# LumiOwO/RT-Octree

Hardware: AMD Instinct MI355X
Metric: FPS @ 800x800 (Lego SPP=6) + PSNR vs ref; 1/2/4/8 GPU scaling (higher is better)
Workload: dtype f32 (traversal, filter) + f16 x f16 -> f32 (GuidanceNet conv, fused MFMA kernel); 1 GPU; configs[1]: lego-like synthetic PlenOctree SH16 (2122333 nodes, depth 10), 800x800 SPP=6 + GuidanceNet(8,32,5,2,4) denoise, 1 step = 12 launch groups of 100 frames, frames sharded frame g -> rank g mod N; tree_nodes=2122333, frames_per_group=100, streams=2, scenes=1, scene_map=pose, filter=factorised, maps=fp16 packed, parallelism=frames x1, lean_outputs=True, lean_level=2, world=1, gpus_visible=1, launcher=none, full=False

## Files before the change

### rt-octree_amd/csrc/host/tree_layout.cpp

```cpp
#include "host/tree_layout.h"

#include <cmath>
#include <cstring>

#include "host/n3tree_host.h"
#include "rto_tree_bits.h"

namespace rto {

float half_to_float(uint16_t h) {
    const uint32_t sign = (uint32_t)(h & 0x8000u) << 16, exp = (h >> 10) & 0x1fu, man = h & 0x3ffu;
    uint32_t bits;
    if (exp == 0) {
        if (man == 0) {
            bits = sign;
        } else {
            int e = -1;
            uint32_t m = man;
            do {
                ++e;
                m <<= 1;
            } while (!(m & 0x400u));
            bits = sign | (uint32_t)(127 - 15 - e) << 23 | (m & 0x3ffu) << 13;
        }
    } else if (exp == 31) {
        bits = sign | 0x7f800000u | man << 13;
    } else {
        bits = sign | (exp + 127 - 15) << 23 | man << 13;
    }
    float f;
    std::memcpy(&f, &bits, 4);
    return f;
}

bool culling_cells(const int32_t* child, int64_t capacity, const float scale[3], const float offset[3], const uint16_t* sigma,
                   size_t stride, std::vector<float>& out) {
    auto density = [&](int64_t sl) { return half_to_float(sigma[(size_t)sl * stride]); };
    std::vector<uint8_t> lvl((size_t)capacity, 255), has((size_t)capacity, 0);
    std::vector<uint32_t> cx((size_t)capacity, 0), cy((size_t)capacity, 0), cz((size_t)capacity, 0);
    lvl[0] = 0;
    for (int64_t n = 0; n < capacity; ++n) {
        if (lvl[(size_t)n] == 255) continue;
        for (int s = 0; s < 8; ++s) {
            const int32_t c = child[n * 8 + s];
            if (c == 0) continue;
            const int64_t t = n + c;
            if (t <= n || t >= capacity || lvl[(size_t)n] >= 30) return false;
            lvl[(size_t)t] = (uint8_t)(lvl[(size_t)n] + 1);
            cx[(size_t)t] = cx[(size_t)n] * 2 + ((s >> 2) & 1);
            cy[(size_t)t] = cy[(size_t)n] * 2 + ((s >> 1) & 1);
            cz[(size_t)t] = cz[(size_t)n] * 2 + (s & 1);
        }
    }
    for (int64_t n = capacity - 1; n >= 0; --n) {
        if (lvl[(size_t)n] == 255) continue;
        uint8_t h = 0;
        for (int s = 0; s < 8 && !h; ++s) {
            const int32_t c = child[n * 8 + s];
            h = c ? has[(size_t)(n + c)] : (uint8_t)(density(n * 8 + s) > 0.f);
        }
        has[(size_t)n] = h;
    }
    out.clear();
    const float margin = 1e-4f;
    for (int64_t n = 0; n < capacity; ++n) {
        if (lvl[(size_t)n] == 255 || !has[(size_t)n]) continue;
        const int ls = lvl[(size_t)n] + 1;
        if (ls > kOccLevel) continue;
        for (int s = 0; s < 8; ++s) {
            const int32_t c = child[n * 8 + s];
            const bool emit = c ? (ls == kOccLevel && has[(size_t)(n + c)]) : density(n * 8 + s) > 0.f;
            if (!emit) continue;
            const double size = std::ldexp(1.0, -ls);
            const uint32_t q[3] = {cx[(size_t)n] * 2 + ((s >> 2) & 1), cy[(size_t)n] * 2 + ((s >> 1) & 1), cz[(size_t)n] * 2 + (s & 1)};
            for (int i = 0; i < 3; ++i) {
                const double ct = (q[i] + 0.5) * size;
                out.push_back((float)((ct - offset[i]) / scale[i]));
            }
            out.push_back((float)(0.5 * size + margin));
        }
    }
    return true;
}

std::vector<int64_t> bfs_order(const int32_t* child, int64_t capacity, int64_t N3) {
    std::vector<int64_t> order;
    order.reserve((size_t)capacity);
    std::vector<uint8_t> seen((size_t)capacity, 0);
    order.push_back(0);
    seen[0] = 1;
    for (size_t h = 0; h < order.size(); ++h) {
        const int64_t o = order[h];
        for (int64_t s = 0; s < N3; ++s) {
            const int32_t c = child[o * N3 + s];
            if (c == 0) continue;
            const int64_t t = o + c;
            if (!seen[(size_t)t]) {
                seen[(size_t)t] = 1;
                order.push_back(t);
            }
        }
    }
    for (int64_t o = 0; o < capacity; ++o)
        if (!seen[(size_t)o]) order.push_back(o);
    return order;
}

void relay_tree(const std::vector<int64_t>& order, const int32_t* child, const uint16_t* data, int64_t capacity, int64_t N3,
                int data_dim, const HostTree* quant, Relaid& out) {
    std::vector<int64_t> new_of_old((size_t)capacity);
    for (int64_t n = 0; n < capacity; ++n) new_of_old[(size_t)order[(size_t)n]] = n;
    out.child.resize((size_t)(capacity * N3));
// ... 156 lines not shown
```

### rt-octree_amd/csrc/host/tree_layout.h

```cpp
#pragma once
#include <cstddef>
#include <cstdint>
#include <vector>

namespace rto {
struct HostTree;
}

#pragma GCC visibility push(hidden)
namespace rto {

float half_to_float(uint16_t h);

bool culling_cells(const int32_t* child, int64_t capacity, const float scale[3], const float offset[3], const uint16_t* sigma,
                   size_t stride, std::vector<float>& out);

std::vector<int64_t> bfs_order(const int32_t* child, int64_t capacity, int64_t N3);

struct Relaid {
    std::vector<int32_t> child;
    std::vector<uint16_t> data, q_map, q_sigma, q_retained;
};
void relay_tree(const std::vector<int64_t>& order, const int32_t* child, const uint16_t* data, int64_t capacity, int64_t N3,
                int data_dim, const HostTree* quant, Relaid& out);

struct WideImage {
    std::vector<uint32_t> widew, worig, gslot;
    uint32_t n_wide = 0, grid_nodes = 0;
};
bool build_wide_image(const int32_t* child, int64_t capacity, int G, const uint16_t* sigma, size_t stride,
                      WideImage& out);

void wide_image_lookup(const WideImage& wi, const int32_t* child, int G, const uint32_t* points, int64_t n, int32_t* out_level,
                       int64_t* out_slot, uint16_t* out_sigma);

}
#pragma GCC visibility pop
```

### rt-octree_amd/csrc/render_kernels.hip

```cpp
#include <hip/hip_runtime.h>

#include "rto_kernel_types.h"
#include "rto_tree_device.h"

#pragma clang fp contract(off)

#include "rto_render_shared.h"
#include "rto_render_internal.h"

namespace rto {



constexpr int kMarkCells = 2048, kMarkLdsWords = 8192;
template <class MarkFn>
RTO_DEV void mark_cell(const float4 cell, const TreeDev& tree, const FrameDesc& fd, const FrameBatch& fb, MarkFn mark);
template <bool LDS_MASK>
__global__ void __launch_bounds__(256) mark_tiles_kernel(const TreeDev tree, const FrameBatch fb, uint32_t* __restrict__ mask) {
    extern __shared__ uint32_t s_mask[];
    const FrameDesc& fd = fb.f[blockIdx.y];
    uint32_t* const gm = mask + (size_t)blockIdx.y * fb.mask_words;
    if (LDS_MASK) {
        for (int i = threadIdx.x; i < fb.mask_words; i += 256) s_mask[i] = 0u;
        __syncthreads();
    }
    static_assert(kMarkCells % 256 == 0, "a run per thread");
    for (int i = 0; i < kMarkCells / 256; ++i) {
        const int c = (int)blockIdx.x * kMarkCells + (int)threadIdx.x * (kMarkCells / 256) + i;
        if (c >= tree.n_occ_cells) break;
        if (LDS_MASK)
            mark_cell(tree.occ_cells[c], tree, fd, fb, [&](uint32_t w, uint32_t bits) { atomicOr(&s_mask[w], bits); });
        else
            mark_cell(tree.occ_cells[c], tree, fd, fb, [&](uint32_t w, uint32_t bits) { atomicOr(gm + w, bits); });
    }
    if (LDS_MASK) {
        __syncthreads();
        for (int i = threadIdx.x; i < fb.mask_words; i += 256)
            if (s_mask[i]) atomicOr(gm + i, s_mask[i]);
    }
}

template <class MarkFn>
RTO_DEV void mark_cell(const float4 cell, const TreeDev& tree, const FrameDesc& fd, const FrameBatch& fb, MarkFn mark) {
    {
    const float* m = fd.transform;
    const float p[3] = {cell.x - m[9], cell.y - m[10], cell.z - m[11]};
    const float c12[3] = {m[4] * m[8] - m[5] * m[7], m[5] * m[6] - m[3] * m[8], m[3] * m[7] - m[4] * m[6]};
    const float c20[3] = {m[7] * m[2] - m[8] * m[1], m[8] * m[0] - m[6] * m[2], m[6] * m[1] - m[7] * m[0]};
    const float c01[3] = {m[1] * m[5] - m[2] * m[4], m[2] * m[3] - m[0] * m[5], m[0] * m[4] - m[1] * m[3]};
    const float det = m[0] * c12[0] + m[1] * c12[1] + m[2] * c12[2];
    const float inv = 1.f / det;
    const float a = (p[0] * c12[0] + p[1] * c12[1] + p[2] * c12[2]) * inv;
    const float b = (p[0] * c20[0] + p[1] * c20[1] + p[2] * c20[2]) * inv;
    const float d = -(p[0] * c01[0] + p[1] * c01[1] + p[2] * c01[2]) * inv;
    const float frob = sqrtf(c12[0] * c12[0] + c12[1] * c12[1] + c12[2] * c12[2] + c20[0] * c20[0] + c20[1] * c20[1] + c20[2] * c20[2] +
                             c01[0] * c01[0] + c01[1] * c01[1] + c01[2] * c01[2]) * fabsf(inv);
    const float hw[3] = {cell.w / fabsf(tree.scale[0]), cell.w / fabsf(tree.scale[1]), cell.w / fabsf(tree.scale[2])};
    const float r = sqrtf(hw[0] * hw[0] + hw[1] * hw[1] + hw[2] * hw[2]) * 1.001f * frob * 1.0001f;
    if (d <= -r) return;
    const float fx = fabsf(fd.fx), fy = fabsf(fd.fy);
    const bool sphere = d > 2.f * r;
    float x0f = 0.f, x1f = 0.f, y0f = 0.f, y1f = 0.f;
    if (sphere) {
        const float xs = a / d, ys = b / d;
        const float k = r / (d - r);
        const float pxc = 0.5f * fb.width + fd.fx * xs, pyc = 0.5f * fb.height - fd.fy * ys;
        const float rx = fx * k * (1.f + fabsf(xs)) + 1.5f, ry = fy * k * (1.f + fabsf(ys)) + 1.5f;
        x0f = floorf((pxc - rx) * 0.125f), x1f = floorf((pxc + rx) * 0.125f);
        y0f = floorf((pyc - ry) * 0.125f), y1f = floorf((pyc + ry) * 0.125f);
    }
    const float ua[3] = {hw[0] * c12[0] * inv, hw[1] * c12[1] * inv, hw[2] * c12[2] * inv};
    const float ub[3] = {hw[0] * c20[0] * inv, hw[1] * c20[1] * inv, hw[2] * c20[2] * inv};
    const float ud[3] = {-hw[0] * c01[0] * inv, -hw[1] * c01[1] * inv, -hw[2] * c01[2] * inv};
    const float e = 1e-5f * ((fabsf(p[0]) + fabsf(p[1]) + fabsf(p[2])) * frob + r);
    const float dmin = 100.f * e;
    bool front = true, behind = true;
    float xlo = 3e38f, xhi = -3e38f, ylo = 3e38f, yhi = -3e38f;
#pragma unroll
    for (int s = 0; s < 8; ++s) {
        const float sx = (s & 4) ? 1.f : -1.f, sy = (s & 2) ? 1.f : -1.f, sz = (s & 1) ? 1.f : -1.f;
        const float A = a + sx * ua[0] + sy * ua[1] + sz * ua[2];
        const float B = b + sx * ub[0] + sy * ub[1] + sz * ub[2];
        const float D = d + sx * ud[0] + sy * ud[1] + sz * ud[2];
        const float x = A / D, y = B / D, k = e / (D - e);
        const float kx = k * (1.f + fabsf(x)), ky = k * (1.f + fabsf(y));
        front = front && D > dmin && fabsf(x) + fabsf(y) < 3e38f;
        behind = behind && D < -e;
        xlo = fminf(xlo, x - kx), xhi = fmaxf(xhi, x + kx);
        ylo = fminf(ylo, y - ky), yhi = fmaxf(yhi, y + ky);
    }
    if (behind) return;
    const float px0 = 0.5f * fb.width + fd.fx * xlo, px1 = 0.5f * fb.width + fd.fx * xhi;
    const float py0 = 0.5f * fb.height - fd.fy * ylo, py1 = 0.5f * fb.height - fd.fy * yhi;
    const bool box = front && fabsf(px0) + fabsf(px1) + fabsf(py0) + fabsf(py1) < 3e38f;
    if (!box && !sphere) {
        mark((uint32_t)fb.mask_words - 1u, 1u);
        return;
    }
    if (box) {
        const float bx0 = floorf((fminf(px0, px1) - 1.5f) * 0.125f), bx1 = floorf((fmaxf(px0, px1) + 1.5f) * 0.125f);
        const float by0 = floorf((fminf(py0, py1) - 1.5f) * 0.125f), by1 = floorf((fmaxf(py0, py1) + 1.5f) * 0.125f);
        x0f = sphere ? fmaxf(x0f, bx0) : bx0, x1f = sphere ? fminf(x1f, bx1) : bx1;
        y0f = sphere ? fmaxf(y0f, by0) : by0, y1f = sphere ? fminf(y1f, by1) : by1;
    }
    const int tiles_x = (fb.width + 7) >> 3, tiles_y = (fb.height + 7) >> 3;
    if (!(x1f >= 0.f && y1f >= 0.f && x0f < (float)tiles_x && y0f < (float)tiles_y)) {
        if (!(x0f == x0f && y0f == y0f)) mark((uint32_t)fb.mask_words - 1u, 1u);
        return;
    }
    const int x0 = x0f < 0.f ? 0 : (int)x0f, x1 = x1f >= (float)tiles_x ? tiles_x - 1 : (int)x1f;
    const int y0 = y0f < 0.f ? 0 : (int)y0f, y1 = y1f >= (float)tiles_y ? tiles_y - 1 : (int)y1f;
    for (int ty = y0; ty <= y1; ++ty)
        for (int tx = x0; tx <= x1; ++tx) {
            const uint32_t t = (uint32_t)(ty * tiles_x + tx);
            mark(t >> 5, 1u << (t & 31u));
        }
    }
}

__global__ void __launch_bounds__(256) mark_tiles_one_kernel(const TreeDev tree, const FrameDesc fd, const int width, const int height,
                                                             const int mask_words, uint32_t* __restrict__ mask) {
    extern __shared__ uint32_t s_mask[];
    FrameBatch fb;
    fb.width = width;
    fb.height = height;
    fb.mask_words = mask_words;
    const bool lds = mask_words <= kMarkLdsWords;
    if (lds) {
        for (int i = threadIdx.x; i < mask_words; i += 256) s_mask[i] = 0u;
        __syncthreads();
    }
    for (int i = 0; i < kMarkCells / 256; ++i) {
        const int c = (int)blockIdx.x * kMarkCells + (int)threadIdx.x * (kMarkCells / 256) + i;
        if (c >= tree.n_occ_cells) break;
        if (lds)
            mark_cell(tree.occ_cells[c], tree, fd, fb, [&](uint32_t w, uint32_t bits) { atomicOr(&s_mask[w], bits); });
        else
            mark_cell(tree.occ_cells[c], tree, fd, fb, [&](uint32_t w, uint32_t bits) { atomicOr(mask + w, bits); });
    }
    if (lds) {
        __syncthreads();
        for (int i = threadIdx.x; i < mask_words; i += 256)
            if (s_mask[i]) atomicOr(mask + i, s_mask[i]);
    }
}

RTO_DEV bool tile_marked(const FrameBatch& fb, int frame, uint32_t tile_index) {
    const uint32_t* fm = fb.tile_mask + (size_t)frame * fb.mask_words;
    return ((fm[tile_index >> 5] >> (tile_index & 31u)) | fm[fb.mask_words - 1]) & 1u;
}

RTO_DEV bool queue_slot(const FrameBatch& fb, int k, uint32_t pt, uint32_t& entry) {
    const uint32_t qt0 = (uint32_t)fb.qstart[k], qtiles = (uint32_t)fb.qstart[k + 1] - qt0, n = (uint32_t)fb.n;
    if (pt >= qtiles * n) return false;
    uint32_t tile, frame;
    if (fb.tile_major) {
        const uint32_t t = pt / n;
        frame = pt - t * n;
        tile = qt0 + t;
    } else {
        frame = pt / qtiles;
        tile = qt0 + (pt - frame * qtiles);
    }
    const uint32_t tiles_x = (uint32_t)(fb.width + 7) >> 3;
    uint32_t tx, ty;
    if (fb.tile_order) {
        const uint32_t code = fb.tile_order[tile];
        ty = code >> 16;
        tx = code & 0xffffu;
    } else {
        ty = tile / tiles_x;
// ... 290 lines not shown
```

### rt-octree_amd/csrc/rto_abi.cpp

```cpp
#include <algorithm>
#include <cmath>
#include <cstdio>
#include <cstring>
#include <fstream>
#include <sstream>

#include "host/mini_json.h"
#include "rto_denoise_launch.h"
#include "rto_internal.h"

namespace {
thread_local std::string g_err;
}

int set_err(int code, const std::string& msg) {
    g_err = msg;
    return code;
}

namespace {

void pcg_seed(rto::Pcg32& r, uint64_t initstate, uint64_t initseq) {
    auto next = [&]() { r.state = r.state * rto::kPcgMult + r.inc; };
    r.state = 0U;
// ... 411 lines not shown
    if (!c || n < 1 || first_slot < 0 || first_slot + n > c->frames) return 0;
    int lean = 0;
    for (int i = first_slot; i < first_slot + n; ++i) lean += c->lean_slot[(size_t)i] ? 1 : 0;
    return lean == n ? 1 : lean == 0 ? 0 : -1;
}

int rto_ctx_set_tuning(rto_ctx* c, const char* key, int value) {
    if (!c || !key) return set_err(RTO_E_INVALID, "rto_ctx_set_tuning: null argument");
    const std::string k(key);
    if (k == "tile_order") {
        c->tile_order_on = value != 0;
    } else if (k == "xcd_queues") {
        c->xcd_queues = value != 0;
    } else if (k == "tile_major") {
        c->tile_major = value != 0;
    } else if (k == "tile_block") {
        if (value < 1 || value > 64) return set_err(RTO_E_INVALID, "tile_block must be 1..64");
        c->tile_block = value;
        DeviceGuard guard(c->device);
        if (hipDeviceSynchronize() != hipSuccess) return set_err(RTO_E_HIP, "hipDeviceSynchronize failed");
        return build_tile_tables(c);
    } else if (k == "queue_bands") {
        if (value < 0 || value > 64) return set_err(RTO_E_INVALID, "queue_bands must be 0..64");
        c->queue_bands = value;
        DeviceGuard guard(c->device);
        if (hipDeviceSynchronize() != hipSuccess) return set_err(RTO_E_HIP, "hipDeviceSynchronize failed");
        return build_tile_tables(c);
    } else if (k == "refill") {
        c->refill = value;
    } else if (k == "wide_bits") {
        c->test_wide_bits = value;
    } else if (k == "cull") {
        c->cull_on = value != 0;
    } else if (k == "cull_single") {
        c->cull_single = value != 0;
    } else if (k == "frame_via_batch") {
        c->frame_via_batch = value != 0;
    } else if (k == "blocks_per_cu") {
        if (value < 0 || value > 8) return set_err(RTO_E_INVALID, "blocks_per_cu must be 0..8");
        c->occ.cap = value;
    } else if (k == "batch_fallback") {
        c->batch_fallback = value;
    } else if (k == "ray_order") {
        if (value < 0 || value > 1) return set_err(RTO_E_INVALID, "ray_order must be 0 or 1");
        c->ray_order = value;
    } else if (k == "strip_rows") {
        if (value < 1) return set_err(RTO_E_INVALID, "strip_rows must be >= 1");
        c->strip_rows = value;
    } else {
        return set_err(RTO_E_INVALID, "unknown tuning key '" + k + "'");
    }
    return RTO_OK;
}

int rto_ctx_kernel_timing(rto_ctx* c, int enable) {
    if (!c) return set_err(RTO_E_INVALID, "rto_ctx_kernel_timing: null context");
    DeviceGuard guard(c->device);
    if (enable && c->kt_ev.empty()) {
        c->kt_ev.resize((size_t)kKtRing * 4);
        for (auto& e : c->kt_ev) HIP_TRY(hipEventCreate(&e));
    }
    c->kt_on = enable != 0;
    c->kt_count = 0;
    return RTO_OK;
}

// ... 255 lines not shown
```

### rt-octree_amd/csrc/rto_internal.h

```cpp
#pragma once
#include <hip/hip_runtime.h>

#include <algorithm>
#include <atomic>
#include <cmath>
#include <cstring>
#include <mutex>
#include <string>
#include <vector>

#include "rto.h"
#include "rto_abi_common.h"
#include "rto_launch.h"

#pragma GCC visibility push(hidden)

constexpr const char* kNoDeviceMsg = "no HIP device available (librto has no CPU fallback)";
constexpr int kKtRing = 256;
constexpr int kProbeFloats = 128;
#pragma GCC visibility pop

struct rto_tree {
    int device = 0;
    rto::TreeDev dev{};
    rto_tree_info info{};
    void* d_data = nullptr;
    void* d_child = nullptr;
    void* d_nodew = nullptr;
    void* d_topgrid = nullptr;
    void *d_widew = nullptr, *d_worig = nullptr, *d_grid2 = nullptr;
    void* d_shrec = nullptr;
    void* d_recidx = nullptr;
    void* d_occ = nullptr;
    void* d_qrec = nullptr;
    void* d_qcolors = nullptr;
    void* d_qsigma = nullptr;
    void* d_extra = nullptr;
    bool quant = false;
    int flags = 0;
    bool fast_ok = false;
    std::atomic<bool> reference_dropped{false};
    int shrec_halves = 0;
    std::mutex rebuild_mutex;
};

#ifndef RTO_QUEUE_BANDS_DEFAULT
#define RTO_QUEUE_BANDS_DEFAULT 3
#endif
#ifndef RTO_RAY_ORDER_DEFAULT
#define RTO_RAY_ORDER_DEFAULT 0
#endif
struct rto_ctx {
    int device = 0;
    int width = 0, height = 0;
    int frames = 1;
    int sel = 0;
    int num_cus = 256;
    unsigned long long* queue = nullptr;
    rto::FrameDesc* d_frames = nullptr;
    rto::OccupancyCache occ;
    uint32_t* tile_order = nullptr;
    uint32_t* wedge_order = nullptr;
    int wedge_start[rto::kMaxQueues + 1] = {0};
    bool xcd_queues = true;
    bool tile_major = true;
    int tile_block = 4;
    int queue_bands = RTO_QUEUE_BANDS_DEFAULT;
    uint32_t* hits = nullptr;
    int hits_spp = 0;
    uint32_t* tile_mask = nullptr;
    uint32_t* qlist = nullptr;
    uint32_t* qscratch = nullptr;
    int mask_words = 0, q_chunks_cap = 0;
    bool cull_on = true;
    bool frame_via_batch = false;
    int last_n_queues = 0;
    int64_t last_slots = 0;
    int batch_fallback = 0;
    int lean = 0;
    std::vector<uint8_t> lean_slot;
    int test_wide_bits = 0;
    bool cull_single = false;
    int marks_n = 0, marks_slot0 = 0;
    float marks_bg = 0.f;
    bool kt_on = false;
    std::vector<hipEvent_t> kt_ev;
    int kt_count = 0;
    float* aux = nullptr;
    float* noisy = nullptr;
    float* image = nullptr;
    const float* layer_depth = nullptr;
    const float* layer_color = nullptr;
    float* depth = nullptr;
    float* t_near = nullptr;
    int depth_mode = 0;
    float* probe_coeffs = nullptr;
    uint8_t* rgba8 = nullptr;
    rto::Pcg32 rng{};
    rto::PcgJumpEntry* jump = nullptr;
    uint64_t jump_inc = 0;
    bool jump_valid = false;
    int kernel = RTO_KERNEL_AUTO;
    int strip_rows = 1;
    int ray_order = RTO_RAY_ORDER_DEFAULT;
    int refill = 0;
    bool tile_order_on = true;
    bool stats_on = false;
// ... 92 lines not shown
```

### rt-octree_amd/csrc/rto_render_abi.cpp

```cpp
#include <algorithm>
#include <cstring>

#include "rto_internal.h"

namespace {

int ensure_jump_table(rto_ctx* c) {
    if (c->jump_valid && c->jump_inc == c->rng.inc) return RTO_OK;
    std::vector<rto::PcgJumpEntry> tab(4 * 256);
    for (int ch = 0; ch < 4; ++ch)
        for (int j = 0; j < 256; ++j) tab[ch * 256 + j] = pcg_jump(c->rng.inc, (uint64_t)j << (8 * ch));
    if (!c->jump) HIP_TRY(hipMalloc((void**)&c->jump, tab.size() * sizeof(rto::PcgJumpEntry)));
    HIP_TRY(hipMemcpy(c->jump, tab.data(), tab.size() * sizeof(rto::PcgJumpEntry), hipMemcpyHostToDevice));
    c->jump_inc = c->rng.inc;
    c->jump_valid = true;
    return RTO_OK;
}


int check_tree_options(const rto_tree* tree, const rto_options* o, const rto_ctx* ctx) {
    if (!spp_supported(o->spp))
        return set_err(RTO_E_SPP, "spp == " + std::to_string(o->spp) + " not supported. (supported: 1,2,3,4,6,8,16,32)");
    if (tree->device != ctx->device) return set_err(RTO_E_INVALID, "tree and context live on different devices");
    if (tree->d_recidx && !(o->sigma_thresh >= 0.f))
// ... 254 lines not shown
    const bool depth_batched = ctx->depth && ctx->depth_mode == RTO_DEPTH_BATCHED;
    const bool batched = spp_supported(o->spp) && fast_path_for_spp(tree, o->spp, ctx->test_wide_bits, &tdev) != 0 &&
                         ctx->batch_fallback != 1 && (!ctx->depth || depth_batched);
    int rc = check_batch(tree, cams, n, o, ctx, slot0, batched);
    if (rc != RTO_OK) return rc;
    DeviceGuard guard(ctx->device);
    if (!guard.ok) return set_err(RTO_E_HIP, "hipSetDevice failed");
    hipStream_t stream = (hipStream_t)stream_;
    if (ctx->depth && !batched) return depth_frames(tree, cams, rng_jumps, n, o, ctx, stream, slot0);
    if (!batched) return generic_frames(tree, cams, rng_jumps, n, o, ctx, stream, slot0);

    ctx->marks_n = 0;
    for (int f = 0; f < n; ++f) ctx->lean_slot[(size_t)(slot0 + f)] = 0;
    const size_t px = frame_px(ctx);
    if (ctx->hits_spp < o->spp) {
        if (ctx->hits) {
            HIP_TRY(hipDeviceSynchronize());
            HIP_TRY(hipFree(ctx->hits));
            ctx->hits = nullptr;
        }
        HIP_TRY(hipMalloc((void**)&ctx->hits, (size_t)ctx->frames * o->spp * px * sizeof(uint32_t)));
        ctx->hits_spp = o->spp;
    }
    rto::FrameBatch fb;
    std::memset(&fb, 0, sizeof(fb));
    fb.n = n;
    fb.width = ctx->width;
    fb.height = ctx->height;
    rc = queue_layout(ctx, n, &fb);
    if (rc != RTO_OK) return rc;
    ctx->last_n_queues = fb.n_queues;
    ctx->last_slots = (int64_t)tiles_of(ctx) * n;
    const bool cull = ctx->cull_on && tree->dev.occ_cells && o->sigma_thresh >= 0.f && !(tree->dev.ndc_width > 0.f);
    rto::FrameDesc frames[rto::kMaxBatch];
    fb.f = ctx->d_frames;
    fb.lean = o->denoise ? ctx->lean : 0;
    for (int f = 0; f < n; ++f) {
        rto::FrameDesc& d = frames[f];
        d.fx = cams[f].fx;
        d.fy = cams[f].fy;
        std::memcpy(d.transform, cams[f].transform, sizeof(d.transform));
        const rto::Pcg32 rng = rng_after(ctx, frame_jump(rng_jumps, f));
        d.rng_state = rng.state;
        d.rng_inc = rng.inc;
        const rto::FrameOut fo = frame_out(ctx, slot0 + f, o->denoise);
        d.aux = fo.aux;
        d.image = fo.image;
        d.hits = ctx->hits + (size_t)(slot0 + f) * o->spp * px;
    }
    rc = ensure_jump_table(ctx);
    if (rc != RTO_OK) return rc;
    const rto::OptDev od = make_opt_dev(o);
    HIP_TRY(rto::launch_write_frames(frames, n, ctx->d_frames, stream));
    hipEvent_t* ev = nullptr;
    if (ctx->kt_on && ctx->kt_count < kKtRing) ev = &ctx->kt_ev[(size_t)ctx->kt_count++ * 4];
    ctx->occ.force_lds_refusal = ctx->batch_fallback == 2;
    rto::LayerDev layers;
    const bool layered = ctx_layers_at(ctx, slot0, &layers);
    rto::DepthOut dout;
    const bool with_depth = ctx_depth_at(ctx, slot0, &dout);
    hipError_t e = rto::launch_render_batch(o->spp, tdev, od, fb, ctx->jump, ctx->queue,
                                            frames[0].hits,
                                            ctx->num_cus, ctx->refill, cull, &ctx->occ, ev, layered ? &layers : nullptr,
                                            with_depth ? &dout : nullptr, stream);
    if (ctx->occ.lds_refused) {
        if (ev) --ctx->kt_count;
// ... 27 lines not shown
    rto::LayerDev layers;
    const bool layered = ctx_layers_at(ctx, ctx->sel, &layers);
    int rc = check_layers(tree, ctx, layered);
    if (rc == RTO_OK) rc = check_depth(tree, o, ctx);
    if (rc != RTO_OK) return rc;
    if (tree->quant) {
        if (ctx->kernel == RTO_KERNEL_GENERIC || ctx->stats_on)
            return set_err(RTO_E_UNSUPPORTED, "a quantised tree loaded with RTO_TREE_QUANT_DIRECT has no generic kernel / work counters");
        return launch_batch_at(tree, cam, nullptr, 1, o, ctx, stream_, ctx->sel);
    }
    rc = check_tree_options(tree, o, ctx);
    if (rc == RTO_OK) rc = check_camera(*cam, ctx);
    if (rc == RTO_OK && o->enable_probe) rc = probe_check(tree, o, ctx, layered);
    int kernel;
    rto::TreeDev tdev;
    if (rc == RTO_OK) rc = choose_kernel(tree, o, ctx, &kernel, &tdev);
    if (rc != RTO_OK) return rc;
    const bool fast = kernel == RTO_KERNEL_FAST;
    if (fast && ctx->frame_via_batch && ctx->kernel == RTO_KERNEL_AUTO && !ctx->stats_on && !ctx->depth)
        return launch_batch_at(tree, cam, nullptr, 1, o, ctx, stream_, ctx->sel);

    DeviceGuard guard(ctx->device);
    if (!guard.ok) return set_err(RTO_E_HIP, "hipSetDevice failed");
    hipStream_t stream = (hipStream_t)stream_;
    rc = fast ? ensure_jump_table(ctx) : ensure_reference_arrays(tree);
    if (rc != RTO_OK) return rc;
    const rto::CamDev cd = cam_dev(*cam);
    rto::FrameOut fo = frame_out(ctx, ctx->sel, o->denoise);
    const bool cull_one = fast && !ctx->stats_on && ctx->cull_on && ctx->cull_single && tree->dev.occ_cells &&
                          o->sigma_thresh >= 0.f && !(tree->dev.ndc_width > 0.f) && !o->enable_probe;
    if (cull_one) {
        rc = ensure_tile_buffers(ctx, mask_words_of(ctx), 0);
        if (rc != RTO_OK) return rc;
        HIP_TRY(rto::launch_mark_tiles_one(tdev, cd, ctx->tile_mask, ctx->mask_words, stream));
        fo.cull_marks = ctx->tile_mask;
        fo.cull_mask_words = ctx->mask_words;
    }
    bool keep_marks = false;
    if (ctx->stats_on) {
        if (!fast) return set_err(RTO_E_UNSUPPORTED, "work counters need the fast kernel");
        fo.stats = ctx->stats;
        if (ctx->stats_marks) {
            if (ctx->marks_n < 1 || !ctx->tile_mask || ctx->sel < ctx->marks_slot0 || ctx->sel >= ctx->marks_slot0 + ctx->marks_n)
                return set_err(RTO_E_INVALID, "rto_ctx_enable_stats(2): the selected frame slot holds no tile marks of a batched launch");
            fo.stat_marks = ctx->tile_mask + (size_t)(ctx->sel - ctx->marks_slot0) * ctx->mask_words;
            fo.stat_mask_words = ctx->mask_words;
            keep_marks = true;
        }
    }
    if (!keep_marks) ctx->marks_n = 0;
    ctx->lean_slot[(size_t)ctx->sel] = 0;
    rto::DepthOut depth;
    const bool with_depth = ctx_depth_at(ctx, ctx->sel, &depth);
    rc = render_frame(tree, fast ? tdev : tree->dev, kernel, cd, o, make_opt_dev(o), ctx->rng, fo, layered ? &layers : nullptr,
                      with_depth ? &depth : nullptr, ctx, stream);
    if (rc != RTO_OK) return rc;
    if (cull_one && !(layered && layers.color)) {
        ctx->marks_n = 1;
        ctx->marks_slot0 = ctx->sel;
        ctx->marks_bg = o->background_brightness;
    }
    return RTO_OK;
}

int rto_launch_renderer_batch(const rto_tree* tree, const rto_camera* cams, const int64_t* rng_jumps, int n,
                              const rto_options* o, rto_ctx* ctx, void* stream_) {
// ... 60 lines not shown
```

### rt-octree_amd/csrc/rto_tree.cpp

```cpp
#include <algorithm>
#include <cmath>
#include <cstdio>
#include <cstdlib>
#include <cstring>

#include "host/n3tree_host.h"
#include "host/tree_layout.h"
#include "rto_internal.h"

namespace {

bool tree_alloc(rto_tree* t, void** p, size_t bytes) {
    if (hipMalloc(p, bytes) != hipSuccess) return false;
    t->info.device_bytes += (int64_t)bytes;
    return true;
}
void tree_release(rto_tree* t, void** p, size_t bytes) {
    if (!*p) return;
    (void)hipFree(*p);
    *p = nullptr;
    t->info.device_bytes -= (int64_t)bytes;
}

struct HostArrays {
// ... 93 lines not shown
                    tree_alloc(t, &t->d_qrec, rec_b) &&
                    rto::launch_pack_quant((const uint16_t*)tmp_map, (const uint16_t*)tmp_ret, n_slots, nr, nq, q_rec,
                                           (uint16_t*)t->d_qrec, nullptr) == hipSuccess &&
                    hipDeviceSynchronize() == hipSuccess;
    if (tmp_map) (void)hipFree(tmp_map);
    if (tmp_ret) (void)hipFree(tmp_ret);
    if (!ok) return set_err(RTO_E_HIP, "quantised tree upload failed");
    t->quant = true;
    t->dev.q_retain = nr;
    t->dev.q_rec = q_rec;
    return RTO_OK;
}

int build_nodew(rto_tree* t, const HostArrays& h) {
    if (!(h.N == 2 && h.max_depth <= 24 && h.n_slots < (int64_t(1) << rto::kGridSlotBits))) return RTO_OK;
    int* d_bad = nullptr;
    if (!tree_alloc(t, &t->d_nodew, (size_t)h.n_slots * 4) || hipMalloc((void**)&d_bad, 4) != hipSuccess ||
        hipMemset(d_bad, 0, 4) != hipSuccess)
        return set_err(RTO_E_HIP, "hipMalloc(nodew) failed");
    const uint16_t* d_sigma = h.quant ? (const uint16_t*)t->d_qsigma : (const uint16_t*)t->d_data;
    hipError_t e = rto::launch_build_nodew((const int32_t*)t->d_child, d_sigma, h.n_slots, h.quant ? 1 : h.data_dim,
                                           (uint32_t*)t->d_nodew, d_bad, nullptr);
    int bad = 0;
    if (e == hipSuccess) e = hipMemcpy(&bad, d_bad, 4, hipMemcpyDeviceToHost);
    (void)hipFree(d_bad);
    if (e != hipSuccess) return hip_fail("build_nodew failed: ", e);
    t->fast_ok = !bad;
    if (bad) tree_release(t, &t->d_nodew, (size_t)h.n_slots * 4);
    return RTO_OK;
}

int upload_culling_cells(rto_tree* t, const HostArrays& h, const float scale[3], const float offset[3]) {
    if (!t->fast_ok || (t->flags & RTO_TREE_NO_CULLING)) return RTO_OK;
    std::vector<float> cells;
    if (!rto::culling_cells(h.child, h.capacity, scale, offset, h.sigma, h.sigma_stride, cells)) return RTO_OK;
    const size_t bytes = cells.empty() ? 16 : cells.size() * sizeof(float);
    if (!tree_alloc(t, &t->d_occ, bytes) ||
        (!cells.empty() && hipMemcpy(t->d_occ, cells.data(), cells.size() * sizeof(float), hipMemcpyHostToDevice) != hipSuccess))
        return set_err(RTO_E_HIP, "hipMalloc(culling cells) failed");
    t->dev.occ_cells = (const float4*)t->d_occ;
    t->dev.n_occ_cells = (int)(cells.size() / 4);
    return RTO_OK;
}

int build_top_grid(rto_tree* t, const HostArrays& h) {
    if (!t->fast_ok || h.max_depth < 3) return RTO_OK;
    int top_levels = h.max_depth - 1 < 6 ? h.max_depth - 1 : 6;
    if (const char* ev = getenv("RTO_TOP_LEVELS")) {
        const int g = atoi(ev);
        if (g >= 3 && g <= 8 && g <= h.max_depth - 1) top_levels = g;
    }
    if (!tree_alloc(t, &t->d_topgrid, (size_t)8 << (3 * top_levels))) return set_err(RTO_E_HIP, "hipMalloc(topgrid) failed");
    hipError_t e = rto::launch_build_topgrid((const uint32_t*)t->d_nodew, top_levels, (uint2*)t->d_topgrid, nullptr);
    if (e == hipSuccess) e = hipDeviceSynchronize();
    if (e != hipSuccess) return hip_fail("build_topgrid failed: ", e);
    t->dev.top_levels = top_levels;
    return RTO_OK;
}

void upload_wide_image(rto_tree* t, const HostArrays& h) {
    if (!t->fast_ok || getenv("RTO_NO_WIDE")) return;
    rto::WideImage wi;
    if (!rto::build_wide_image(h.child, h.capacity, t->dev.top_levels, h.sigma, h.sigma_stride, wi)) return;
    const size_t wb = wi.widew.size() * 4, ob = wi.worig.size() * 4, gb = wi.gslot.size() * 4;
    const bool up = tree_alloc(t, &t->d_widew, wb) && tree_alloc(t, &t->d_worig, ob) && tree_alloc(t, &t->d_grid2, gb) &&
                    hipMemcpy(t->d_widew, wi.widew.data(), wb, hipMemcpyHostToDevice) == hipSuccess &&
                    hipMemcpy(t->d_worig, wi.worig.data(), ob, hipMemcpyHostToDevice) == hipSuccess &&
                    hipMemcpy(t->d_grid2, wi.gslot.data(), gb, hipMemcpyHostToDevice) == hipSuccess;
    if (!up) {
        (void)hipGetLastError();
        tree_release(t, &t->d_widew, wb);
        tree_release(t, &t->d_worig, ob);
        tree_release(t, &t->d_grid2, gb);
        return;
// ... 327 lines not shown
    } else if (data_dim == 4) {
        fmt.format = RTO_FMT_RGBA;
        fmt.basis_dim = -1;
    } else {
        fmt.format = RTO_FMT_SH;
        fmt.basis_dim = (data_dim - 1) / 3;
    }
    return upload_tree(child, data, capacity, N, data_dim, fmt, scale, offset, device, out, nullptr, flags & ~RTO_TREE_QUANT_DIRECT,
                       extra, extra_floats);
}

int rto_tree_set_ndc(rto_tree* t, float w, float h, float focal) {
    if (!t) return set_err(RTO_E_INVALID, "rto_tree_set_ndc: null tree");
    t->info.use_ndc = w > 0;
    t->info.ndc_width = w;
    t->info.ndc_height = h;
    t->info.ndc_focal = focal;
    t->dev.ndc_width = w > 0 ? w : -1.f;
    t->dev.ndc_height = h;
    t->dev.ndc_focal = focal;
    return RTO_OK;
}

int rto_tree_get_info(const rto_tree* t, rto_tree_info* info) {
    if (!t || !info) return set_err(RTO_E_INVALID, "rto_tree_get_info: null argument");
    *info = t->info;
    return RTO_OK;
}

void rto_tree_free(rto_tree* t) {
    if (!t) return;
    DeviceGuard guard(t->device);
    for (void* p : {t->d_data, t->d_child, t->d_nodew, t->d_topgrid, t->d_widew, t->d_worig, t->d_grid2, t->d_shrec, t->d_recidx, t->d_occ,
                    t->d_qrec, t->d_qcolors, t->d_qsigma, t->d_extra})
        if (p) (void)hipFree(p);
    delete t;
}

int rto_probe_basis(const rto_tree* tree, const rto_options* o, const float* dirs, int64_t n, int path, float* host_out) {
    if (!tree || !o || !dirs || !host_out || n <= 0 || (path != 0 && path != 1))
        return set_err(RTO_E_INVALID, "rto_probe_basis: null argument, n <= 0 or path not 0 / 1");
    if (missing_lobes(tree)) return set_err(RTO_E_FORMAT, missing_lobes_msg);
    if (n > (int64_t(1) << 31) - 256) return set_err(RTO_E_INVALID, "rto_probe_basis: n above 2^31 - 256");
    DeviceGuard guard(tree->device);
    if (!guard.ok) return set_err(RTO_E_HIP, "hipSetDevice failed");
    const rto::OptDev od = make_opt_dev(o);
    const size_t in_b = (size_t)n * 3 * sizeof(float), out_b = (size_t)n * RTO_BASIS_MAX * sizeof(float);
    float *d_dirs = nullptr, *d_out = nullptr;
    hipError_t e = hipMalloc((void**)&d_dirs, in_b);
    if (e == hipSuccess) e = hipMalloc((void**)&d_out, out_b);
    if (e == hipSuccess) e = hipMemcpy(d_dirs, dirs, in_b, hipMemcpyHostToDevice);
    bool no_form = false;
    if (e == hipSuccess) {
        e = rto::launch_probe_basis(tree->dev, od, d_dirs, n, path, d_out, nullptr);
        no_form = e == hipErrorInvalidValue;
    }
    if (e == hipSuccess) e = hipMemcpy(host_out, d_out, out_b, hipMemcpyDeviceToHost);
    if (d_dirs) (void)hipFree(d_dirs);
    if (d_out) (void)hipFree(d_out);
    if (no_form) {
        rto::DataFormat fmt;
        fmt.format = tree->dev.format;
        fmt.basis_dim = tree->dev.basis_dim;
        return set_err(RTO_E_UNSUPPORTED, "rto_probe_basis: the shading kernel has no per-B form for " + fmt.to_string());
    }
    if (e != hipSuccess) return set_err(RTO_E_HIP, std::string("rto_probe_basis: ") + hipGetErrorString(e));
    return RTO_OK;
// ... 90 lines not shown
```

Before: 16430 frames/s.

## Cull tiles with tight per-cell occupied bounding boxes and smaller pad

Culling cells now carry a tight axis-aligned bound of the occupied sub-region, computed bottom-up over the octree in fixed-point, instead of the full cube. The mark kernel reads a center plus per-axis half-extents, and the screen-space tile pad drops from 1.5 to 0.5 pixels, so fewer tiles get marked and fewer rays are traced. The cell buffer doubles in size, and a second cube buffer is kept for an opt-in fallback. A smaller pad risks dropping edge tiles and slightly changing the image.

```diff
diff --git a/rt-octree_amd/csrc/host/tree_layout.cpp b/rt-octree_amd/csrc/host/tree_layout.cpp
--- a/rt-octree_amd/csrc/host/tree_layout.cpp
+++ b/rt-octree_amd/csrc/host/tree_layout.cpp
@@ -34,10 +34,12 @@
 }
 
 bool culling_cells(const int32_t* child, int64_t capacity, const float scale[3], const float offset[3], const uint16_t* sigma,
-                   size_t stride, std::vector<float>& out) {
+                   size_t stride, std::vector<float>& out, std::vector<float>* cubes) {
     auto density = [&](int64_t sl) { return half_to_float(sigma[(size_t)sl * stride]); };
     std::vector<uint8_t> lvl((size_t)capacity, 255), has((size_t)capacity, 0);
     std::vector<uint32_t> cx((size_t)capacity, 0), cy((size_t)capacity, 0), cz((size_t)capacity, 0);
+    constexpr uint32_t kHalf = 1u << 30;
+    std::vector<uint32_t> blo((size_t)capacity * 3, 0), bhi((size_t)capacity * 3, 0);
     lvl[0] = 0;
     for (int64_t n = 0; n < capacity; ++n) {
         if (lvl[(size_t)n] == 255) continue;
@@ -55,13 +57,24 @@
     for (int64_t n = capacity - 1; n >= 0; --n) {
         if (lvl[(size_t)n] == 255) continue;
         uint8_t h = 0;
-        for (int s = 0; s < 8 && !h; ++s) {
+        uint32_t lo[3] = {2 * kHalf, 2 * kHalf, 2 * kHalf}, hi[3] = {0, 0, 0};
+        for (int s = 0; s < 8; ++s) {
             const int32_t c = child[n * 8 + s];
-            h = c ? has[(size_t)(n + c)] : (uint8_t)(density(n * 8 + s) > 0.f);
+            if (!(c ? has[(size_t)(n + c)] : (uint8_t)(density(n * 8 + s) > 0.f))) continue;
+            h = 1;
+            const uint32_t bit[3] = {(uint32_t)(s >> 2) & 1u, (uint32_t)(s >> 1) & 1u, (uint32_t)s & 1u};
+            for (int i = 0; i < 3; ++i) {
+                const uint32_t l = bit[i] * kHalf + (c ? blo[(size_t)(n + c) * 3 + i] >> 1 : 0u);
+                const uint32_t u = bit[i] * kHalf + (c ? bhi[(size_t)(n + c) * 3 + i] >> 1 : kHalf);
+                lo[i] = l < lo[i] ? l : lo[i];
+                hi[i] = u > hi[i] ? u : hi[i];
+            }
         }
         has[(size_t)n] = h;
+        for (int i = 0; i < 3 && h; ++i) blo[(size_t)n * 3 + i] = lo[i], bhi[(size_t)n * 3 + i] = hi[i];
     }
     out.clear();
+    if (cubes) cubes->clear();
     const float margin = 1e-4f;
     for (int64_t n = 0; n < capacity; ++n) {
         if (lvl[(size_t)n] == 255 || !has[(size_t)n]) continue;
@@ -73,11 +86,16 @@
             if (!emit) continue;
             const double size = std::ldexp(1.0, -ls);
             const uint32_t q[3] = {cx[(size_t)n] * 2 + ((s >> 2) & 1), cy[(size_t)n] * 2 + ((s >> 1) & 1), cz[(size_t)n] * 2 + (s & 1)};
+            float box[8] = {0.f}, cube[8] = {0.f};
             for (int i = 0; i < 3; ++i) {
-                const double ct = (q[i] + 0.5) * size;
-                out.push_back((float)((ct - offset[i]) / scale[i]));
-            }
-            out.push_back((float)(0.5 * size + margin));
+                const double l = c ? std::ldexp((double)blo[(size_t)(n + c) * 3 + i], -31) : 0.0;
+                const double u = c ? std::ldexp((double)bhi[(size_t)(n + c) * 3 + i], -31) : 1.0;
+                box[i] = (float)(((q[i] + 0.5 * (l + u)) * size - offset[i]) / scale[i]);
+                box[4 + i] = (float)(0.5 * (u - l) * size + margin);
+                cube[i] = (float)(((q[i] + 0.5) * size - offset[i]) / scale[i]);
+                cube[4 + i] = (float)(0.5 * size + margin);
+            }            out.insert(out.end(), box, box + 8);
+            if (cubes) cubes->insert(cubes->end(), cube, cube + 8);
         }
     }
     return true;
diff --git a/rt-octree_amd/csrc/host/tree_layout.h b/rt-octree_amd/csrc/host/tree_layout.h
--- a/rt-octree_amd/csrc/host/tree_layout.h
+++ b/rt-octree_amd/csrc/host/tree_layout.h
@@ -13,7 +13,7 @@
 float half_to_float(uint16_t h);
 
 bool culling_cells(const int32_t* child, int64_t capacity, const float scale[3], const float offset[3], const uint16_t* sigma,
-                   size_t stride, std::vector<float>& out);
+                   size_t stride, std::vector<float>& out, std::vector<float>* cubes = nullptr);
 
 std::vector<int64_t> bfs_order(const int32_t* child, int64_t capacity, int64_t N3);
 
diff --git a/rt-octree_amd/csrc/render_kernels.hip b/rt-octree_amd/csrc/render_kernels.hip
--- a/rt-octree_amd/csrc/render_kernels.hip
+++ b/rt-octree_amd/csrc/render_kernels.hip
@@ -13,8 +13,12 @@
 
 
 constexpr int kMarkCells = 2048, kMarkLdsWords = 8192;
+#ifndef RTO_MARK_PAD
+#define RTO_MARK_PAD 0.5f
+#endif
+constexpr float kMarkPad = RTO_MARK_PAD;
 template <class MarkFn>
-RTO_DEV void mark_cell(const float4 cell, const TreeDev& tree, const FrameDesc& fd, const FrameBatch& fb, MarkFn mark);
+RTO_DEV void mark_cell(const float4 cell, const float4 half, const TreeDev& tree, const FrameDesc& fd, const FrameBatch& fb, MarkFn mark);
 template <bool LDS_MASK>
 __global__ void __launch_bounds__(256) mark_tiles_kernel(const TreeDev tree, const FrameBatch fb, uint32_t* __restrict__ mask) {
     extern __shared__ uint32_t s_mask[];
@@ -29,9 +33,9 @@
         const int c = (int)blockIdx.x * kMarkCells + (int)threadIdx.x * (kMarkCells / 256) + i;
         if (c >= tree.n_occ_cells) break;
         if (LDS_MASK)
-            mark_cell(tree.occ_cells[c], tree, fd, fb, [&](uint32_t w, uint32_t bits) { atomicOr(&s_mask[w], bits); });
+            mark_cell(tree.occ_cells[2 * c], tree.occ_cells[2 * c + 1], tree, fd, fb, [&](uint32_t w, uint32_t bits) { atomicOr(&s_mask[w], bits); });
         else
-            mark_cell(tree.occ_cells[c], tree, fd, fb, [&](uint32_t w, uint32_t bits) { atomicOr(gm + w, bits); });
+            mark_cell(tree.occ_cells[2 * c], tree.occ_cells[2 * c + 1], tree, fd, fb, [&](uint32_t w, uint32_t bits) { atomicOr(gm + w, bits); });
     }
     if (LDS_MASK) {
         __syncthreads();
@@ -41,7 +45,7 @@
 }
 
 template <class MarkFn>
-RTO_DEV void mark_cell(const float4 cell, const TreeDev& tree, const FrameDesc& fd, const FrameBatch& fb, MarkFn mark) {
+RTO_DEV void mark_cell(const float4 cell, const float4 half, const TreeDev& tree, const FrameDesc& fd, const FrameBatch& fb, MarkFn mark) {
     {
     const float* m = fd.transform;
     const float p[3] = {cell.x - m[9], cell.y - m[10], cell.z - m[11]};
@@ -55,7 +59,7 @@
     const float d = -(p[0] * c01[0] + p[1] * c01[1] + p[2] * c01[2]) * inv;
     const float frob = sqrtf(c12[0] * c12[0] + c12[1] * c12[1] + c12[2] * c12[2] + c20[0] * c20[0] + c20[1] * c20[1] + c20[2] * c20[2] +
                              c01[0] * c01[0] + c01[1] * c01[1] + c01[2] * c01[2]) * fabsf(inv);
-    const float hw[3] = {cell.w / fabsf(tree.scale[0]), cell.w / fabsf(tree.scale[1]), cell.w / fabsf(tree.scale[2])};
+    const float hw[3] = {half.x / fabsf(tree.scale[0]), half.y / fabsf(tree.scale[1]), half.z / fabsf(tree.scale[2])};
     const float r = sqrtf(hw[0] * hw[0] + hw[1] * hw[1] + hw[2] * hw[2]) * 1.001f * frob * 1.0001f;
     if (d <= -r) return;
     const float fx = fabsf(fd.fx), fy = fabsf(fd.fy);
@@ -98,8 +102,8 @@
         return;
     }
     if (box) {
-        const float bx0 = floorf((fminf(px0, px1) - 1.5f) * 0.125f), bx1 = floorf((fmaxf(px0, px1) + 1.5f) * 0.125f);
-        const float by0 = floorf((fminf(py0, py1) - 1.5f) * 0.125f), by1 = floorf((fmaxf(py0, py1) + 1.5f) * 0.125f);
+        const float bx0 = floorf((fminf(px0, px1) - kMarkPad) * 0.125f), bx1 = floorf((fmaxf(px0, px1) + kMarkPad) * 0.125f);
+        const float by0 = floorf((fminf(py0, py1) - kMarkPad) * 0.125f), by1 = floorf((fmaxf(py0, py1) + kMarkPad) * 0.125f);
         x0f = sphere ? fmaxf(x0f, bx0) : bx0, x1f = sphere ? fminf(x1f, bx1) : bx1;
         y0f = sphere ? fmaxf(y0f, by0) : by0, y1f = sphere ? fminf(y1f, by1) : by1;
     }
@@ -134,9 +138,9 @@
         const int c = (int)blockIdx.x * kMarkCells + (int)threadIdx.x * (kMarkCells / 256) + i;
         if (c >= tree.n_occ_cells) break;
         if (lds)
-            mark_cell(tree.occ_cells[c], tree, fd, fb, [&](uint32_t w, uint32_t bits) { atomicOr(&s_mask[w], bits); });
+            mark_cell(tree.occ_cells[2 * c], tree.occ_cells[2 * c + 1], tree, fd, fb, [&](uint32_t w, uint32_t bits) { atomicOr(&s_mask[w], bits); });
         else
-            mark_cell(tree.occ_cells[c], tree, fd, fb, [&](uint32_t w, uint32_t bits) { atomicOr(mask + w, bits); });
+            mark_cell(tree.occ_cells[2 * c], tree.occ_cells[2 * c + 1], tree, fd, fb, [&](uint32_t w, uint32_t bits) { atomicOr(mask + w, bits); });
     }
     if (lds) {
         __syncthreads();
diff --git a/rt-octree_amd/csrc/rto_abi.cpp b/rt-octree_amd/csrc/rto_abi.cpp
--- a/rt-octree_amd/csrc/rto_abi.cpp
+++ b/rt-octree_amd/csrc/rto_abi.cpp
@@ -467,6 +467,8 @@
         c->test_wide_bits = value;
     } else if (k == "cull") {
         c->cull_on = value != 0;
+    } else if (k == "cull_cubes") {
+        c->cull_cubes = value != 0;
     } else if (k == "cull_single") {
         c->cull_single = value != 0;
     } else if (k == "frame_via_batch") {
diff --git a/rt-octree_amd/csrc/rto_internal.h b/rt-octree_amd/csrc/rto_internal.h
--- a/rt-octree_amd/csrc/rto_internal.h
+++ b/rt-octree_amd/csrc/rto_internal.h
@@ -32,6 +32,7 @@
     void* d_shrec = nullptr;
     void* d_recidx = nullptr;
     void* d_occ = nullptr;
+    void* d_occ_cubes = nullptr;
     void* d_qrec = nullptr;
     void* d_qcolors = nullptr;
     void* d_qsigma = nullptr;
@@ -73,6 +74,7 @@
     uint32_t* qscratch = nullptr;
     int mask_words = 0, q_chunks_cap = 0;
     bool cull_on = true;
+    bool cull_cubes = false;
     bool frame_via_batch = false;
     int last_n_queues = 0;
     int64_t last_slots = 0;
diff --git a/rt-octree_amd/csrc/rto_render_abi.cpp b/rt-octree_amd/csrc/rto_render_abi.cpp
--- a/rt-octree_amd/csrc/rto_render_abi.cpp
+++ b/rt-octree_amd/csrc/rto_render_abi.cpp
@@ -310,6 +310,7 @@
     ctx->last_n_queues = fb.n_queues;
     ctx->last_slots = (int64_t)tiles_of(ctx) * n;
     const bool cull = ctx->cull_on && tree->dev.occ_cells && o->sigma_thresh >= 0.f && !(tree->dev.ndc_width > 0.f);
+    if (ctx->cull_cubes && tree->d_occ_cubes) tdev.occ_cells = (const float4*)tree->d_occ_cubes;
     rto::FrameDesc frames[rto::kMaxBatch];
     fb.f = ctx->d_frames;
     fb.lean = o->denoise ? ctx->lean : 0;
@@ -403,6 +404,7 @@
     if (cull_one) {
         rc = ensure_tile_buffers(ctx, mask_words_of(ctx), 0);
         if (rc != RTO_OK) return rc;
+        if (ctx->cull_cubes && tree->d_occ_cubes) tdev.occ_cells = (const float4*)tree->d_occ_cubes;
         HIP_TRY(rto::launch_mark_tiles_one(tdev, cd, ctx->tile_mask, ctx->mask_words, stream));
         fo.cull_marks = ctx->tile_mask;
         fo.cull_mask_words = ctx->mask_words;
diff --git a/rt-octree_amd/csrc/rto_tree.cpp b/rt-octree_amd/csrc/rto_tree.cpp
--- a/rt-octree_amd/csrc/rto_tree.cpp
+++ b/rt-octree_amd/csrc/rto_tree.cpp
@@ -149,14 +149,15 @@
 
 int upload_culling_cells(rto_tree* t, const HostArrays& h, const float scale[3], const float offset[3]) {
     if (!t->fast_ok || (t->flags & RTO_TREE_NO_CULLING)) return RTO_OK;
-    std::vector<float> cells;
-    if (!rto::culling_cells(h.child, h.capacity, scale, offset, h.sigma, h.sigma_stride, cells)) return RTO_OK;
-    const size_t bytes = cells.empty() ? 16 : cells.size() * sizeof(float);
-    if (!tree_alloc(t, &t->d_occ, bytes) ||
-        (!cells.empty() && hipMemcpy(t->d_occ, cells.data(), cells.size() * sizeof(float), hipMemcpyHostToDevice) != hipSuccess))
-        return set_err(RTO_E_HIP, "hipMalloc(culling cells) failed");
+    std::vector<float> cells, cubes;
+    if (!rto::culling_cells(h.child, h.capacity, scale, offset, h.sigma, h.sigma_stride, cells, &cubes)) return RTO_OK;
+    const size_t bytes = cells.empty() ? 32 : cells.size() * sizeof(float);
+    auto up = [&](void** dst, const std::vector<float>& src) {
+        return tree_alloc(t, dst, bytes) && (src.empty() || hipMemcpy(*dst, src.data(), bytes, hipMemcpyHostToDevice) == hipSuccess);
+    };
+    if (!up(&t->d_occ, cells) || !up(&t->d_occ_cubes, cubes)) return set_err(RTO_E_HIP, "hipMalloc(culling cells) failed");
     t->dev.occ_cells = (const float4*)t->d_occ;
-    t->dev.n_occ_cells = (int)(cells.size() / 4);
+    t->dev.n_occ_cells = (int)(cells.size() / 8);
     return RTO_OK;
 }
 
@@ -550,7 +551,7 @@
     if (!t) return;
     DeviceGuard guard(t->device);
     for (void* p : {t->d_data, t->d_child, t->d_nodew, t->d_topgrid, t->d_widew, t->d_worig, t->d_grid2, t->d_shrec, t->d_recidx, t->d_occ,
-                    t->d_qrec, t->d_qcolors, t->d_qsigma, t->d_extra})
+                    t->d_occ_cubes, t->d_qrec, t->d_qcolors, t->d_qsigma, t->d_extra})
         if (p) (void)hipFree(p);
     delete t;
 }
```

Measured after the change: 16640 frames/s, median of 6. 1.3% higher.
